# ctlab/metafast

Hardware: AMD Instinct MI355X
Metric: k-mers/s counted+graphed at k=31, 150 bp reads (higher is better)
Workload: dtype u64

## Files before the change

metafast_amd/csrc/mf_cc.hip:

```cpp
#include "mf_common.h"
#include "mf_nbr.h"
#include "mf_cc.h"
#include <algorithm>
#include <numeric>
#include <memory>

#define CC_NONE 0xFFFFFFFFu

__global__ void k_cc_adjacency(mf_index_view ix, const uint64_t *__restrict__ keys, uint64_t n,
                               int k, uint32_t *__restrict__ nbr) {
    uint64_t v = (uint64_t)blockIdx.x * blockDim.x + threadIdx.x;
    if (v >= n) return;
    const uint64_t kmask = (1ull << (2 * k)) - 1;
    const uint64_t x = keys[v];
    uint32_t out[8];
    uint32_t m_nf = 0, m_nl = 0;
    if (ix.skm_k) mf_skm_nbr_mins(x, k, &m_nf, &m_nl);
#pragma unroll
    for (uint32_t nuc = 0; nuc < 4; nuc++) {
        uint32_t idx, val;
        uint64_t y = ((x << 2) | nuc) & kmask;
        out[2 * nuc] = mf_index_find_ph(ix, mf_canon(y, k), ix.skm_k ? mf_skm_ph_right(y, k, m_nf) : 0u, &idx, &val) ? idx : CC_NONE;
        y = (x >> 2) | ((uint64_t)nuc << (2 * k - 2));
        out[2 * nuc + 1] = mf_index_find_ph(ix, mf_canon(y, k), ix.skm_k ? mf_skm_ph_left(y, k, m_nl) : 0u, &idx, &val) ? idx : CC_NONE;
    }
    uint4 *o = reinterpret_cast<uint4 *>(nbr + v * 8);
    o[0] = make_uint4(out[0], out[1], out[2], out[3]);
    o[1] = make_uint4(out[4], out[5], out[6], out[7]);
}

template <int MODE, int KT = 0>
__attribute__((amdgpu_waves_per_eu(KT ? 6 : 5, 8)))
__global__ __launch_bounds__(64 * NB_WAVES) void k_cc_adjacency_part(mf_index_view ix, const uint64_t *__restrict__ keys, const uint64_t *__restrict__ part_off,
                                                                   uint32_t np, int k_rt, uint32_t *__restrict__ nbr) {
    __shared__ nb_lds S;
    const int k = KT ? KT : k_rt;
    nb_for_each<MODE>(ix, keys, part_off, 0u, np, k, S, 0, 0u, [&](uint64_t v, uint64_t, const uint32_t (&idx)[8], uint32_t, uint32_t, bool have) {
        if (!have) return;
        uint4 *o = reinterpret_cast<uint4 *>(nbr + v * 8);
        o[0] = make_uint4(idx[0], idx[1], idx[2], idx[3]);
        o[1] = make_uint4(idx[4], idx[5], idx[6], idx[7]);
    });
}

__device__ __forceinline__ uint32_t cc_find(uint32_t *parent, uint32_t x) {
    for (;;) {
        uint32_t p = __hip_atomic_load(&parent[x], __ATOMIC_RELAXED, __HIP_MEMORY_SCOPE_AGENT);
        if (p == x) return x;
        uint32_t gp = __hip_atomic_load(&parent[p], __ATOMIC_RELAXED, __HIP_MEMORY_SCOPE_AGENT);
        if (gp != p) __hip_atomic_store(&parent[x], gp, __ATOMIC_RELAXED, __HIP_MEMORY_SCOPE_AGENT);
        x = gp;
    }
}
#define CC_TILE 1024
#define CC_LEDGE 2048
__global__ __launch_bounds__(256) void k_cc_hook_tile(const uint32_t *__restrict__ nbr, const uint8_t *__restrict__ alive, uint32_t *__restrict__ parent,
                                                      uint32_t *__restrict__ csize, unsigned long long *__restrict__ cweight, uint64_t n,
                                                      uint2 *__restrict__ edges, unsigned long long *__restrict__ ecount, uint64_t ecap) {
    __shared__ uint32_t lp[CC_TILE];
    __shared__ uint8_t la[CC_TILE];
    __shared__ uint2 le[CC_LEDGE];
    __shared__ uint32_t ln;
    __shared__ unsigned long long lbase;
    const uint64_t base = (uint64_t)blockIdx.x * CC_TILE;
    if (threadIdx.x == 0) ln = 0;
    for (uint32_t i = threadIdx.x; i < CC_TILE; i += blockDim.x) {
        lp[i] = i;
        const uint8_t al = base + i < n ? alive[base + i] : 0;
        la[i] = al;
        if (al) { csize[base + i] = 0; cweight[base + i] = 0; }
    }
    __syncthreads();
    auto find_l = [&](uint32_t x) -> uint32_t {
        for (;;) {
            const uint32_t p = *(volatile uint32_t *)&lp[x];
            if (p == x) return x;
            const uint32_t gp = *(volatile uint32_t *)&lp[p];
            if (gp != p) *(volatile uint32_t *)&lp[x] = gp;
            x = gp;
        }
    };
    for (uint32_t i = threadIdx.x; i < CC_TILE; i += blockDim.x) {
        if (!la[i]) continue;
        const uint64_t v = base + i;
        const uint4 *q = reinterpret_cast<const uint4 *>(nbr + v * 8);
        const uint4 a = q[0], b = q[1];
        const uint32_t nb[8] = {a.x, a.y, a.z, a.w, b.x, b.y, b.z, b.w};
#pragma unroll
        for (int j = 0; j < 8; j++) {
            const uint32_t u = nb[j];
            if (u == CC_NONE || u >= (uint32_t)v) continue;
            if (u < (uint32_t)base) {
                if (edges) { const uint32_t e = atomicAdd(&ln, 1u); if (e < (uint32_t)CC_LEDGE) le[e] = make_uint2((uint32_t)v, u); }
                continue;
// ... 797 lines not shown
        out[(size_t)i * n_samples + i] = 0.0;
        for (int j = i + 1; j < n_samples; j++) {
            double sumdiff = 0, sum = 0;
            const int64_t *a = vecs + (size_t)i * n_comp, *b = vecs + (size_t)j * n_comp;
            for (int p = 0; p < n_comp; p++) {
                double x = (double)a[p], y = (double)b[p];
                sumdiff += x > y ? x - y : y - x;
                sum += (x < 0 ? -x : x) + (y < 0 ? -y : y);
            }
            out[(size_t)i * n_samples + j] = out[(size_t)j * n_samples + i] = sumdiff / sum;
        }
    }
    return MF_OK;
}

struct dcc_query { uint64_t key; uint64_t src; };
struct dcc_kept_rec { uint32_t g, size; unsigned long long weight; };
#define DCC_NOKEY 0x7FFFFFFFFFFFFFFFull
struct mf_dcc {
    mf_ctx *ctx = nullptr; mf_table *t = nullptr; int k = 0, rank = 0, world = 1, lw = 0;
    uint32_t n = 0, n_total = 0; std::vector<uint32_t> base;
    mf_buf<uint32_t> nbr, parent, root, csize, groot;
    mf_buf<unsigned long long> cweight; mf_buf<uint8_t> alive;
    mf_buf<uint2> edges; mf_buf<unsigned long long> ecount; uint64_t ecap = 0;
    mf_buf<unsigned int> ctr;
    std::vector<uint64_t> qoff;
    mf_buf<unsigned long long> qcur;
    mf_buf<dcc_query> qflat; uint32_t nq = 0;
    mf_buf<uint32_t> xv, xu; mf_buf<uint8_t> xr, xalive; mf_buf<uint16_t> xval; uint64_t nx = 0;
    std::vector<uint64_t> xoff;
    mf_buf<uint32_t> pg, gsize; mf_buf<unsigned long long> gweight, gmin;
    mf_buf<uint64_t> mk; mf_buf<uint32_t> mg; uint64_t nm = 0;
    uint64_t nstat = 0, nkept_owned = 0; int level = 0;
    mf_buf<uint32_t> touched; mf_buf<uint2> hp; std::vector<uint64_t> xstart;
    mf_buf<dcc_kept_rec> keptbuf;
    mf_buf<uint64_t> gmk; mf_buf<uint2> gruns; uint64_t n_runs = 0;
    mf_buf<uint64_t> dseg; mf_buf<uint32_t> dbase;
};


static int dcc_log2(int w) { int l = 0; while ((1 << l) < w) l++; return l; }
#define DCC_SRC_MASK ((1ull << 56) - 1ull)
#define DCC_QCHUNK 512u
template <int MODE>
__global__ __launch_bounds__(64 * NB_WAVES) void k_dcc_adjacency_part(mf_index_view ix, const uint64_t *__restrict__ keys, const uint64_t *__restrict__ part_off,
                                                                    uint32_t p_lo, uint32_t p_hi, int k, int lw, uint32_t me, uint32_t *__restrict__ nbr,
                                                                    dcc_query *__restrict__ q, uint32_t qcap, unsigned int *__restrict__ qcount) {
    __shared__ nb_lds S;
    const uint64_t kmask = (1ull << (2 * k)) - 1;
    uint32_t qcur = 0, qend = 0;
    auto void_rest = [&]() {
        for (uint32_t i = qcur + mf_lane(); i < qend; i += 64) if (i < qcap) q[i].src = ~0ull;
    };
    nb_for_each<MODE>(ix, keys, part_off, p_lo, p_hi, k, S, lw, me, [&](uint64_t v, uint64_t x, const uint32_t (&idx)[8], uint32_t, uint32_t foreign, bool have) {
        if (have) {
            uint4 *o = reinterpret_cast<uint4 *>(nbr + v * 8);
            o[0] = make_uint4(idx[0], idx[1], idx[2], idx[3]);
            o[1] = make_uint4(idx[4], idx[5], idx[6], idx[7]);
        }
        const uint32_t cnt = have ? (uint32_t)__popc(foreign) : 0u;
        uint32_t tot;
        const uint32_t ex = mf_wave_excl_scan(cnt, &tot);
        if (!tot) return;
        if (qcur + tot > qend) {
            void_rest();
            uint32_t base = 0;
            const uint32_t ch = tot > DCC_QCHUNK ? tot : DCC_QCHUNK;
            if (mf_lane() == 0) base = atomicAdd(qcount, ch);
            qcur = (uint32_t)__builtin_amdgcn_readfirstlane((int)base);
            qend = qcur + ch;
        }
        uint32_t at = qcur + ex;
        qcur += tot;
        if (cnt) {
            uint32_t m_nf = 0, m_nl = 0;
            mf_skm_nbr_mins(x, k, &m_nf, &m_nl);
#pragma unroll
            for (uint32_t i = 0; i < 8; i++) {
                if (!((foreign >> i) & 1u)) continue;
                uint64_t y; uint32_t ph;
                const uint64_t c = nb_neighbour(x, k, kmask, i, m_nf, m_nl, &y, &ph);
                if (at < qcap) { q[at].key = c; q[at].src = (v * 8 + i) | ((uint64_t)(ph >> (32 - lw)) << 56); }
                at++;
            }
        }
    });
    void_rest();
}
template <bool FILL>
__global__ __launch_bounds__(256) void k_dcc_q_group(const dcc_query *__restrict__ q, uint32_t n, unsigned long long *__restrict__ cur, dcc_query *__restrict__ out) {
    __shared__ uint32_t cnt[64]; __shared__ unsigned long long base[64];
    if (threadIdx.x < 64) cnt[threadIdx.x] = 0;
    __syncthreads();
    const uint32_t per = 256 * 8, i0 = blockIdx.x * per;
    uint32_t o[8], pos[8];
#pragma unroll
    for (int j = 0; j < 8; j++) {
        const uint32_t i = i0 + (uint32_t)j * 256u + threadIdx.x;
        o[j] = 0xFFFFFFFFu;
        if (i < n) { o[j] = (uint32_t)(q[i].src >> 56); if (o[j] < 64u) pos[j] = atomicAdd(&cnt[o[j]], 1u); else o[j] = 0xFFFFFFFFu; }
    }
    __syncthreads();
    if (threadIdx.x < 64 && cnt[threadIdx.x]) base[threadIdx.x] = atomicAdd(&cur[threadIdx.x], (unsigned long long)cnt[threadIdx.x]);
    if (!FILL) return;
    __syncthreads();
#pragma unroll
    for (int j = 0; j < 8; j++) {
        const uint32_t i = i0 + (uint32_t)j * 256u + threadIdx.x;
        if (o[j] == 0xFFFFFFFFu) continue;
        dcc_query r = q[i];
        r.src &= DCC_SRC_MASK;
        out[base[o[j]] + pos[j]] = r;
    }
}
struct dcc_answer { uint64_t src; uint32_t lid; uint32_t val; };
__global__ void k_dcc_answer(mf_index_view ix, const dcc_query *__restrict__ q, uint64_t n, dcc_answer *__restrict__ a) {
    const uint64_t i = (uint64_t)blockIdx.x * blockDim.x + threadIdx.x;
    if (i >= n) return;
    uint32_t idx, val;
    const bool f = ix.slots && mf_index_find(ix, q[i].key, &idx, &val);
    a[i].src = q[i].src; a[i].lid = f ? idx : CC_NONE; a[i].val = f ? val : 0u;
}
__device__ __forceinline__ uint64_t dcc_reserve_by(unsigned long long *cur, uint32_t r, bool act, uint32_t *L) {
    unsigned long long *base = reinterpret_cast<unsigned long long *>(L + 64);
    __syncthreads();
    if (threadIdx.x < 64) L[threadIdx.x] = 0;
    __syncthreads();
    uint32_t pos = 0;
    if (act) pos = atomicAdd(&L[r], 1u);
    __syncthreads();
    if (threadIdx.x < 64 && L[threadIdx.x]) base[threadIdx.x] = atomicAdd(&cur[threadIdx.x], (unsigned long long)L[threadIdx.x]);
    __syncthreads();
    return act ? base[r] + pos : 0ull;
}
// ... 764 lines not shown
```

metafast_amd/csrc/mf_common.h:

```cpp
#pragma once
#include <hip/hip_runtime.h>
#include <stdint.h>
#include <stdarg.h>
#include <stdio.h>
#include <string.h>
#include <map>
#include <string>
#include <vector>
#include "../../include/metafast_hip.h"

int mf_set_error(const char *fmt, ...);

#define MF_HIP(call)                                                                              \
    do {                                                                                          \
        hipError_t e__ = (call);                                                                  \
        if (e__ != hipSuccess)                                                                    \
            return mf_set_error("%s failed: %s (%s:%d)", #call, hipGetErrorString(e__), __FILE__, \
                                __LINE__);                                                        \
    } while (0)
#define MF_TRY(call)                  \
    do {                              \
        int r__ = (call);             \
        if (r__ < 0) return r__;      \
    } while (0)
// ... 289 lines not shown
}

__device__ __forceinline__ uint32_t mf_block_excl_scan(uint32_t v, uint32_t *scratch, uint32_t *block_total) {
    uint32_t wtot;
    uint32_t ex = mf_wave_excl_scan(v, &wtot);
    int wave = threadIdx.x >> 6, nw = blockDim.x >> 6;
    __syncthreads();
    if (mf_lane() == 0) scratch[wave] = wtot;
    __syncthreads();
    if (threadIdx.x == 0) {
        uint32_t acc = 0;
        for (int i = 0; i < nw; i++) { uint32_t t = scratch[i]; scratch[i] = acc; acc += t; }
        scratch[16] = acc;
    }
    __syncthreads();
    uint32_t r = ex + scratch[wave];
    *block_total = scratch[16];
    return r;
}

__device__ __forceinline__ uint32_t mf_block_reserve(unsigned int *counter, uint32_t mine, uint32_t *scratch) {
    uint32_t tot;
    const uint32_t ex = mf_block_excl_scan(mine, scratch, &tot);
    if (threadIdx.x == 0) scratch[17] = tot ? atomicAdd(counter, tot) : 0u;
    __syncthreads();
    return scratch[17] + ex;
}

__host__ __device__ constexpr int mf_skm_m(int k) { return k <= 25 ? 13 : 15; }
#define MF_SKM_MIN_K 20
#define MF_SKM_BASES 50
__device__ __forceinline__ uint32_t mf_mmer_rc(uint32_t f, int M) {
    uint32_t r = __brev(~f);
    r = ((r & 0xAAAAAAAAu) >> 1) | ((r & 0x55555555u) << 1);
    return r >> (32 - 2 * M);
}
__host__ __device__ constexpr uint32_t mf_mmer_seed(int M) { return M == 13 ? 0x00B9107Fu : 0x051E6720u; }
__device__ __forceinline__ uint32_t mf_mmer_hash(uint32_t canon, int M) { return (canon ^ mf_mmer_seed(M)) * 0x9E3779B1u; }
__device__ __forceinline__ uint32_t mf_remix32(uint32_t h) { h ^= h >> 16; h *= 0x85EBCA6Bu; h ^= h >> 13; h *= 0xC2B2AE35u; return h ^ (h >> 16); }
__device__ __forceinline__ uint32_t mf_skm_ph(uint64_t key, int k) {
    const int M = mf_skm_m(k);
    const uint32_t mm = (1u << (2 * M)) - 1u;
    uint32_t f = (uint32_t)(key >> (2 * (k - M))) & mm, r = mf_mmer_rc(f, M);
    uint32_t best = mf_mmer_hash(f < r ? f : r, M);
    for (int j = k - M - 1; j >= 0; j--) {
        const uint32_t b = (uint32_t)(key >> (2 * j)) & 3u;
        f = ((f << 2) | b) & mm;
        r = (r >> 2) | ((3u - b) << (2 * M - 2));
        const uint32_t h = mf_mmer_hash(f < r ? f : r, M);
        best = h < best ? h : best;
    }
    return mf_remix32(best);
}
__device__ __forceinline__ void mf_skm_nbr_mins(uint64_t x, int k, uint32_t *no_first, uint32_t *no_last, uint32_t *own = nullptr) {
    const int M = mf_skm_m(k);
    const uint32_t mm = (1u << (2 * M)) - 1u;
    uint32_t f = (uint32_t)(x >> (2 * (k - M))) & mm, r = mf_mmer_rc(f, M);
    uint32_t h = mf_mmer_hash(f < r ? f : r, M);
    uint32_t a = 0xFFFFFFFFu, b = h;
    for (int j = k - M - 1; j >= 0; j--) {
        const uint32_t c = (uint32_t)(x >> (2 * j)) & 3u;
        f = ((f << 2) | c) & mm;
        r = (r >> 2) | ((3u - c) << (2 * M - 2));
        h = mf_mmer_hash(f < r ? f : r, M);
        a = h < a ? h : a;
        if (j > 0) b = h < b ? h : b;
    }
    *no_first = a; *no_last = b;
    if (own) *own = h < b ? h : b;
}
__device__ __forceinline__ uint32_t mf_skm_mn_right(uint64_t y, int k, uint32_t no_first_of_x) {
    const int M = mf_skm_m(k);
    const uint32_t f = (uint32_t)y & ((1u << (2 * M)) - 1u), r = mf_mmer_rc(f, M);
    const uint32_t h = mf_mmer_hash(f < r ? f : r, M);
    return h < no_first_of_x ? h : no_first_of_x;
}
__device__ __forceinline__ uint32_t mf_skm_mn_left(uint64_t y, int k, uint32_t no_last_of_x) {
    const int M = mf_skm_m(k);
    const uint32_t f = (uint32_t)(y >> (2 * (k - M))) & ((1u << (2 * M)) - 1u), r = mf_mmer_rc(f, M);
    const uint32_t h = mf_mmer_hash(f < r ? f : r, M);
    return h < no_last_of_x ? h : no_last_of_x;
}
__device__ __forceinline__ uint32_t mf_skm_ph_right(uint64_t y, int k, uint32_t no_first_of_x) { return mf_remix32(mf_skm_mn_right(y, k, no_first_of_x)); }
__device__ __forceinline__ uint32_t mf_skm_ph_left(uint64_t y, int k, uint32_t no_last_of_x) { return mf_remix32(mf_skm_mn_left(y, k, no_last_of_x)); }
struct mf_slot { uint64_t key; uint32_t idx; uint32_t val; };
int mf_sort_pairs(mf_ctx *ctx, const uint64_t *d_keys_in, const uint16_t *d_vals_in, uint64_t n, int key_bits, uint64_t *d_keys_out,
                  uint16_t *d_vals_out);
int mf_sort_u32_pairs(mf_ctx *ctx, const uint32_t *d_keys_in, const uint32_t *d_vals_in, uint64_t n, int bits, uint32_t *d_keys_out,
                      uint32_t *d_vals_out);
int mf_sort_u32_u64(mf_ctx *ctx, const uint32_t *d_keys_in, const uint64_t *d_vals_in, uint64_t n, int bits, uint32_t *d_keys_out,
                    uint64_t *d_vals_out);
int mf_sort_u64_u32(mf_ctx *ctx, const uint64_t *d_keys_in, const uint32_t *d_vals_in, uint64_t n, int bits, uint64_t *d_keys_out, uint32_t *d_vals_out);
int mf_sort_u64_u64(mf_ctx *ctx, const uint64_t *d_keys_in, const uint64_t *d_vals_in, uint64_t n, int bits, uint64_t *d_keys_out, uint64_t *d_vals_out);
int mf_sort_u64_u64_pingpong(mf_ctx *ctx, uint64_t *k0, uint64_t *v0, uint64_t n, int first_bit, int bits, uint64_t *k1, uint64_t *v1, int *in_second);
int mf_sort_u64_u64_range(mf_ctx *ctx, const uint64_t *d_keys_in, const uint64_t *d_vals_in, uint64_t n, int first_bit, int bits, uint64_t *d_keys_out, uint64_t *d_vals_out);
int mf_select_by(mf_ctx *ctx, const uint64_t *keys, const uint16_t *sel, const uint16_t *vals, uint64_t n, int thr, mf_buf<uint64_t> &ok,
                 mf_buf<uint16_t> &oc, uint64_t *n_out);
int mf_sum_counts(mf_ctx *ctx, const uint16_t *d_counts, uint64_t n, uint64_t *total);
int mf_table_load_kmers_sum(mf_ctx *ctx, const char *const *files, int nfiles, int freq_threshold, int k, mf_table **out, uint64_t *freq_sum);
int mf_sort_kmers_by_comp(mf_ctx *ctx, const uint32_t *d_comp, const uint64_t *d_kmers, uint64_t n, int key_bits, uint32_t n_comps,
                          uint64_t *d_out);
__host__ __device__ __forceinline__ uint64_t mf_interior(uint64_t x, uint64_t rcx, int k) {
    const uint64_t WM = (1ull << (2 * k - 4)) - 1ull;
    const uint64_t w = (x >> 2) & WM, rw = (rcx >> 2) & WM;
    return w < rw ? w : rw;
}
__host__ __device__ __forceinline__ uint64_t mf_cidx_hkey(uint64_t key, uint32_t skm_k) {
    return skm_k >= 3u ? mf_interior(key, mf_revcomp(key, (int)skm_k), (int)skm_k) : key;
}
__device__ __forceinline__ bool mf_index_find_ph(const mf_index_view &ix, uint64_t key, uint32_t ph, uint32_t *idx, uint32_t *val) {
    if (ix.compact) {
        const uint64_t h = mf_phash(mf_cidx_hkey(key, ix.skm_k));
        const uint64_t part = ix.skm_k ? (uint64_t)(ph >> (32 - ix.part_bits)) : (h >> (64 - ix.part_bits));
        const ulonglong2 d = *reinterpret_cast<const ulonglong2 *>(&ix.dir[2 * part]);
        const uint32_t *__restrict__ reg = reinterpret_cast<const uint32_t *>(ix.slots) + (d.x >> 6);
        const uint32_t rmask = (1u << (uint32_t)(d.x & 63ull)) - 1u, hs = mf_pslot(h), tag = hs >> MF_CIDX_REL_BITS;
        uint32_t s = hs & rmask;
        for (;;) {
            const uint32_t v = reg[s];
            if (v == MF_CIDX_EMPTY) return false;
            if ((v >> MF_CIDX_REL_BITS) == tag) {
                const uint64_t i = d.y + (uint64_t)(v & ((1u << MF_CIDX_REL_BITS) - 1u));
// ... 169 lines not shown
```

metafast_amd/csrc/mf_nbr.h:

```cpp
#pragma once
#include "mf_common.h"
#ifdef __HIPCC__
#define NB_SLOTS 1024
#define NB_CAP 352
#define NB_WAVES 4
#define NB_NONE 0xFFFFFFFFu

#define NB_RQ 64
struct nb_lds {
    uint64_t key[NB_WAVES][NB_CAP];
    uint64_t rq_pa[NB_WAVES][NB_RQ], rq_pb[NB_WAVES][NB_RQ];
    uint32_t rq_mn[NB_WAVES][NB_RQ], rq_meta[NB_WAVES][NB_RQ];
    uint32_t slot[NB_WAVES][NB_SLOTS / 2];
};

__device__ __forceinline__ uint64_t nb_neighbour(uint64_t x, uint64_t rcx, int k, uint64_t kmask, uint32_t i, uint32_t m_nf, uint32_t m_nl, uint64_t *oriented, uint32_t *ph) {
    const uint32_t nuc = i >> 1;
    uint64_t y, r;
    if (i & 1u) { y = (x >> 2) | ((uint64_t)nuc << (2 * k - 2)); r = ((rcx << 2) | (uint64_t)(3u - nuc)) & kmask; *ph = mf_skm_ph_left(y, k, m_nl); }
    else { y = ((x << 2) | nuc) & kmask; r = (rcx >> 2) | ((uint64_t)(3u - nuc) << (2 * k - 2)); *ph = mf_skm_ph_right(y, k, m_nf); }
    *oriented = y;
    return y < r ? y : r;
}
__device__ __forceinline__ uint64_t nb_neighbour(uint64_t x, int k, uint64_t kmask, uint32_t i, uint32_t m_nf, uint32_t m_nl, uint64_t *oriented, uint32_t *ph) {
    return nb_neighbour(x, mf_revcomp(x, k), k, kmask, i, m_nf, m_nl, oriented, ph);
}
#define NB_BIGCAP (NB_CAP * NB_WAVES)
__device__ __forceinline__ uint32_t nb_hash(uint64_t key) { return ((uint32_t)key ^ (uint32_t)(key >> 29)) * 0x9E3779B1u; }
__device__ __forceinline__ uint64_t nb_interior(uint64_t x, uint64_t rcx, int k) {
    const uint64_t WM = (1ull << (2 * k - 4)) - 1ull;
    const uint64_t w = (x >> 2) & WM, rw = (rcx >> 2) & WM;
    return w < rw ? w : rw;
}
template <int MODE, typename F>
__device__ __forceinline__ void nb_for_each(const mf_index_view &ix, const uint64_t *__restrict__ keys, const uint64_t *__restrict__ part_off,
                                            uint32_t p_lo, uint32_t np, int k, nb_lds &S, int lw, uint32_t me, F &&emit) {
    constexpr bool BIG = MODE == 2;
    constexpr uint32_t SLOTS = BIG ? (uint32_t)(NB_SLOTS * NB_WAVES) : (uint32_t)NB_SLOTS;
    constexpr int HSHIFT = BIG ? 20 : 22;
    constexpr int POSBITS = BIG ? 11 : 9;
    constexpr uint32_t POSMASK = (1u << POSBITS) - 1u;
    constexpr int TSHIFT = HSHIFT - (16 - POSBITS);
    constexpr uint32_t TAGMASK = (1u << (16 - POSBITS)) - 1u;
    const uint32_t wave = threadIdx.x >> 6, lane = threadIdx.x & 63u;
    const uint32_t first = BIG ? blockIdx.x : blockIdx.x * NB_WAVES + wave, stride = BIG ? gridDim.x : gridDim.x * NB_WAVES;
    const uint64_t kmask = (1ull << (2 * k)) - 1;
    uint64_t *hk = BIG ? &S.key[0][0] : S.key[wave]; uint32_t *hw = BIG ? &S.slot[0][0] : S.slot[wave];
    const uint16_t *hs = reinterpret_cast<const uint16_t *>(hw);
    uint64_t *qa = S.rq_pa[wave], *qb = S.rq_pb[wave]; uint32_t *qm = S.rq_mn[wave], *qt = S.rq_meta[wave];
    const uint32_t tl = BIG ? threadIdx.x : lane, tn = BIG ? (uint32_t)(64 * NB_WAVES) : 64u;
    auto wave_sync = [&]() { __builtin_amdgcn_fence(__ATOMIC_RELEASE, "wavefront"); __builtin_amdgcn_wave_barrier(); __builtin_amdgcn_fence(__ATOMIC_ACQUIRE, "wavefront"); };
    auto team_sync = [&]() { if (BIG) __syncthreads(); else wave_sync(); };
    for (uint32_t p = p_lo + first; p < np; p += stride) {
        const uint64_t lo = part_off[p], hi = part_off[p + 1];
        const uint32_t n = (uint32_t)(hi - lo);
        if (n == 0) continue;
        const bool mid = n > (uint32_t)NB_CAP && n <= (uint32_t)NB_BIGCAP;
        if (MODE == 1 && mid) continue;
        if (MODE == 2 && !mid) continue;
        const bool local = BIG || n <= (uint32_t)NB_CAP;
        if (local) {
            for (uint32_t s = tl; s < SLOTS / 2; s += tn) hw[s] = 0xFFFFFFFFu;
            team_sync();
            for (uint32_t j = tl; j < n; j += tn) {
                const uint64_t x = keys[lo + j];
                hk[j] = x;
                const uint32_t h = nb_hash(nb_interior(x, mf_revcomp(x, k), k));
                const uint32_t ent = (((h >> TSHIFT) & TAGMASK) << POSBITS) | j;
                uint32_t s = h >> HSHIFT;
                for (;;) {
                    uint32_t *w = &hw[s >> 1];
                    const uint32_t sh = (s & 1u) * 16u;
                    const uint32_t old = __atomic_load_n(w, __ATOMIC_RELAXED);
                    if (((old >> sh) & 0xFFFFu) != 0xFFFFu) { s = (s + 1u) & (SLOTS - 1u); continue; }
                    if (atomicCAS(w, old, (old & ~(0xFFFFu << sh)) | (ent << sh)) == old) break;
                }
            }
            team_sync();
        }
        constexpr uint32_t JSTEP = BIG ? (uint32_t)(64 * NB_WAVES) : 64u;
        for (uint32_t j0 = BIG ? wave * 64u : 0u; j0 < n; j0 += JSTEP) {
            const uint32_t j = j0 + lane;
            const bool have = j < n;
            const uint64_t x = have ? (local ? hk[j] : keys[lo + j]) : 0ull;
            uint32_t m_nf = 0, m_nl = 0, m_own = 0;
            mf_skm_nbr_mins(x, k, &m_nf, &m_nl, &m_own);
            uint32_t remote = 0, foreign = 0, flip = 0;
            uint32_t phs[8];
            const uint64_t rcx = mf_revcomp(x, k);
            const int M = mf_skm_m(k);
            const uint32_t MM = (1u << (2 * M)) - 1u;
#pragma unroll
            for (uint32_t i = 0; i < 8; i++) {
                const uint32_t nuc = i >> 1;
                const uint32_t f = (i & 1u) ? (((uint32_t)(x >> (2 * (k - M) + 2)) & (MM >> 2)) | (nuc << (2 * M - 2))) : ((((uint32_t)x << 2) | nuc) & MM);
                const uint32_t r = mf_mmer_rc(f, M), h = mf_mmer_hash(f < r ? f : r, M), mo = (i & 1u) ? m_nl : m_nf;
                phs[i] = h < mo ? h : mo;
                if (have && lw && (mf_remix32(phs[i]) >> (32 - lw)) != me) foreign |= 1u << i;
                else if (have && !(local && phs[i] == m_own)) remote |= 1u << i;
            }
            uint32_t lead[2], grouped = 0, nreq = 0;
#pragma unroll
            for (uint32_t side = 0; side < 2; side++) {
                const uint32_t rem = (remote >> side) & 0x55u;
                lead[side] = 0;
                bool same = true;
#pragma unroll
                for (int c = 3; c >= 0; c--) if ((rem >> (2 * c)) & 1u) lead[side] = phs[2 * c + side];
#pragma unroll
                for (uint32_t c = 0; c < 4; c++) if (((rem >> (2 * c)) & 1u) && phs[2 * c + side] != lead[side]) same = false;
                if (same) grouped |= 1u << side;
                nreq += rem ? (same ? 1u : (uint32_t)__popc(rem)) : 0u;
            }
            uint32_t R;
            const uint32_t rbase = mf_wave_excl_scan(nreq, &R);
            uint32_t idx[8];
#pragma unroll
            for (uint32_t i = 0; i < 8; i++) idx[i] = NB_NONE;
            {
                const uint64_t LM = kmask >> 2;
                uint32_t at = rbase;
#pragma unroll
                for (uint32_t side = 0; side < 2; side++) {
                    const uint32_t rem = (remote >> side) & 0x55u;
                    if (!rem) continue;
                    const uint64_t pa = side ? (rcx & LM) : (x & LM), pb = side ? (x >> 2) : (rcx >> 2);
                    uint32_t want4 = 0;
#pragma unroll
                    for (uint32_t c = 0; c < 4; c++) want4 |= ((rem >> (2 * c)) & 1u) << c;
                    if ((grouped >> side) & 1u) {
                        if (at < (uint32_t)NB_RQ) { qa[at] = pa; qb[at] = pb; qm[at] = lead[side]; qt[at] = side | (want4 << 1); }
                        else {
                            uint32_t o4[4], rv;
                            mf_index_walk_side(ix, mf_remix32(lead[side]), pa, pb, side, want4, k, o4, &rv);
#pragma unroll
                            for (uint32_t c = 0; c < 4; c++) if ((want4 >> c) & 1u) { idx[2 * c + side] = o4[c]; flip |= ((rv >> c) & 1u) << (2 * c + side); }
                        }
                        at++;
                    } else {
#pragma unroll
                        for (uint32_t c = 0; c < 4; c++) {
                            if (!((want4 >> c) & 1u)) continue;
                            if (at < (uint32_t)NB_RQ) { qa[at] = pa; qb[at] = pb; qm[at] = phs[2 * c + side]; qt[at] = side | (1u << (c + 1)); }
                            else { uint32_t o4[4], rv; mf_index_walk_side(ix, mf_remix32(phs[2 * c + side]), pa, pb, side, 1u << c, k, o4, &rv); idx[2 * c + side] = o4[c]; flip |= ((rv >> c) & 1u) << (2 * c + side); }
                            at++;
                        }
                    }
                }
            }
            static_assert(NB_RQ <= 64, "one request per lane");
            const uint32_t Rl = R < (uint32_t)NB_RQ ? R : (uint32_t)NB_RQ;
            ulonglong2 dent = make_ulonglong2(0ull, 0ull);
            if (R) {
                wave_sync();
                if (lane < Rl && ix.compact) dent = mf_index_side_dir(ix, mf_remix32(qm[lane]));
            }
            if (local) {
                const uint64_t LM = kmask >> 2, WM = kmask >> 4;
                const uint32_t nloc = ~(remote | foreign);
#pragma unroll
                for (uint32_t side = 0; side < 2; side++) {
                    if (have && (nloc & (0x55u << side))) {
                        const uint64_t w = side ? (x >> 4) : (x & WM), rw = side ? (rcx & WM) : (rcx >> 4);
                        const uint64_t pa = side ? (rcx & LM) : (x & LM);
                        const uint64_t pb = side ? (x >> 2) : (rcx >> 2);
                        const uint32_t h = nb_hash(w < rw ? w : rw), tag = (h >> TSHIFT) & TAGMASK;
                        uint32_t s = h >> HSHIFT;
                        for (;;) {
                            const uint32_t v = hs[s];
                            if (v == 0xFFFFu) break;
                            if ((v >> POSBITS) == tag) {
                                const uint64_t K = hk[v & POSMASK];
                                const bool ma = (K >> 2) == pa, mb = (K & LM) == pb, fwd = side ? mb : ma;
                                const uint32_t ca = ((uint32_t)K & 3u) ^ (side ? 3u : 0u), cb = (uint32_t)(K >> (2 * k - 2)) ^ (side ? 0u : 3u);
                                const uint32_t c = (ma || mb) ? (fwd ? (side ? cb : ca) : (side ? ca : cb)) : 4u;
                                const uint32_t at = (uint32_t)lo + (v & POSMASK);
#pragma unroll
                                for (uint32_t q = 0; q < 4; q++)
                                    if (c == q && ((nloc >> (2 * q + side)) & 1u)) { idx[2 * q + side] = at; flip = (flip & ~(1u << (2 * q + side))) | ((fwd ? 0u : 1u) << (2 * q + side)); }
                            }
                            s = (s + 1u) & (SLOTS - 1u);
                        }
                    }
                }
            }
            if (R) {
                if (lane < Rl) {
                    uint32_t o4[4], rv = 0;
                    const uint32_t meta = qt[lane];
                    if (ix.compact) mf_index_walk_side_d(ix, dent, qa[lane], qb[lane], meta & 1u, meta >> 1, k, o4, &rv);
                    else mf_index_walk_side(ix, mf_remix32(qm[lane]), qa[lane], qb[lane], meta & 1u, meta >> 1, k, o4, &rv);
                    uint32_t *ans = reinterpret_cast<uint32_t *>(&qa[lane]), *ans2 = reinterpret_cast<uint32_t *>(&qb[lane]);
                    ans[0] = o4[0]; ans[1] = o4[1]; ans2[0] = o4[2]; ans2[1] = o4[3]; qt[lane] = rv;
                }
                wave_sync();
                uint32_t at = rbase;
#pragma unroll
                for (uint32_t side = 0; side < 2; side++) {
                    const uint32_t rem = (remote >> side) & 0x55u;
                    if (!rem) continue;
#pragma unroll
                    for (uint32_t c = 0; c < 4; c++) {
                        if (!((rem >> (2 * c)) & 1u)) continue;
                        if (at < (uint32_t)NB_RQ) {
                            idx[2 * c + side] = c < 2 ? reinterpret_cast<const uint32_t *>(&qa[at])[c] : reinterpret_cast<const uint32_t *>(&qb[at])[c - 2];
                            flip |= ((qt[at] >> c) & 1u) << (2 * c + side);
                        }
                        if (!((grouped >> side) & 1u)) at++;
                    }
                    if ((grouped >> side) & 1u) at++;
                }
                wave_sync();
            }
            emit(lo + j, x, idx, flip, foreign, have);
        }
        team_sync();
    }
}
#endif
```

metafast_amd/csrc/mf_unitig.hip:

```cpp
#include "mf_common.h"
#include "mf_nbr.h"
#include "mf_unitig.h"
#include "mf_wide.h"
#include <algorithm>
#include <numeric>

#define UT_NONE 0xFFFFFFFFu
#define UT_CODE_NONE 4u
#define UT_CODE_MANY 5u
#define UT_WALK_CHUNK 4096

__global__ void k_ut_flags(mf_index_view ix, ut_arrays A) {
    uint64_t i = (uint64_t)blockIdx.x * blockDim.x + threadIdx.x;
    if (i >= A.n) return;
    const int k = A.k;
    const uint64_t kmask = (k == 32) ? ~0ull : ((1ull << (2 * k)) - 1);
    const uint64_t x = A.gk[i];
    uint32_t rcode = UT_CODE_NONE, lcode = UT_CODE_NONE, ridx = UT_NONE, lidx = UT_NONE, ror = 0, lor = 0;
    uint32_t m_nf = 0, m_nl = 0;
    if (ix.skm_k) mf_skm_nbr_mins(x, k, &m_nf, &m_nl);
#pragma unroll
    for (uint32_t nuc = 0; nuc < 4; nuc++) {
        uint64_t y = ((x << 2) | nuc) & kmask;
        uint64_t ry = mf_revcomp(y, k);
        uint64_t c = y < ry ? y : ry;
        uint32_t idx, val;
        if (mf_index_find_ph(ix, c, ix.skm_k ? mf_skm_ph_right(y, k, m_nf) : 0u, &idx, &val)) {
            if (rcode == UT_CODE_NONE) { rcode = nuc; ridx = idx; ror = (c != y); }
            else rcode = UT_CODE_MANY;
        }
    }
#pragma unroll
    for (uint32_t nuc = 0; nuc < 4; nuc++) {
        uint64_t y = (x >> 2) | ((uint64_t)nuc << (2 * k - 2));
        uint64_t ry = mf_revcomp(y, k);
        uint64_t c = y < ry ? y : ry;
        uint32_t idx, val;
        if (mf_index_find_ph(ix, c, ix.skm_k ? mf_skm_ph_left(y, k, m_nl) : 0u, &idx, &val)) {
            if (lcode == UT_CODE_NONE) { lcode = nuc; lidx = idx; lor = (c != y); }
            else lcode = UT_CODE_MANY;
        }
    }
    A.info[i] = (uint8_t)(rcode | (lcode << 3) | (ror << 6) | (lor << 7));
    if (A.pal) A.pal[i] = (uint8_t)(mf_revcomp(x, k) == x);
    A.ridx[i] = ridx;
    A.lidx[i] = lidx;
}

template <int MODE, int KT = 0>
#ifndef NB_NOFORCE
__attribute__((amdgpu_waves_per_eu((KT == 0 || KT == 25 || KT == 29) ? 5 : 6, 8)))
#endif
__global__ __launch_bounds__(64 * NB_WAVES) void k_ut_flags_part(mf_index_view ix, ut_arrays A, const uint64_t *__restrict__ part_off, uint32_t np) {
    __shared__ nb_lds S;
    const int k = KT ? KT : A.k;
    nb_for_each<MODE>(ix, A.gk, part_off, 0u, np, k, S, 0, 0u, [&](uint64_t i, uint64_t x, const uint32_t (&idx)[8], uint32_t flip, uint32_t, bool have) {
        if (!have) return;
        uint32_t rcode = UT_CODE_NONE, lcode = UT_CODE_NONE, ridx = UT_NONE, lidx = UT_NONE, ror = 0, lor = 0;
#pragma unroll
        for (uint32_t nuc = 0; nuc < 4; nuc++) {
            if (idx[2 * nuc] != NB_NONE) {
                if (rcode == UT_CODE_NONE) { rcode = nuc; ridx = idx[2 * nuc]; ror = (flip >> (2 * nuc)) & 1u; }
                else rcode = UT_CODE_MANY;
            }
            if (idx[2 * nuc + 1] != NB_NONE) {
                if (lcode == UT_CODE_NONE) { lcode = nuc; lidx = idx[2 * nuc + 1]; lor = (flip >> (2 * nuc + 1)) & 1u; }
                else lcode = UT_CODE_MANY;
            }
        }
        A.info[i] = (uint8_t)(rcode | (lcode << 3) | (ror << 6) | (lor << 7));
        if (A.pal) A.pal[i] = (uint8_t)(mf_revcomp(x, k) == x);
        A.ridx[i] = ridx;
        A.lidx[i] = lidx;
    });
}

__device__ __forceinline__ bool ut_r_unique(uint8_t info, uint32_t o) { return ((o ? (info >> 3) : info) & 7u) < 4u; }
__device__ __forceinline__ bool ut_l_unique(uint8_t info, uint32_t o) { return ((o ? info : (info >> 3)) & 7u) < 4u; }
__device__ __forceinline__ uint32_t ut_node(const ut_arrays &A, uint32_t idx, uint32_t strand) {
    if (A.pal && A.pal[idx]) strand = 0;
    return idx * 2u + strand;
}
__device__ __forceinline__ uint32_t ut_right_node(const ut_arrays &A, uint32_t i, uint32_t o, uint8_t info) {
    return o ? ut_node(A, A.lidx[i], ((info >> 7) & 1u) ^ 1u) : ut_node(A, A.ridx[i], (info >> 6) & 1u);
}
__device__ __forceinline__ uint32_t ut_left_node(const ut_arrays &A, uint32_t i, uint32_t o, uint8_t info) {
    return o ? ut_node(A, A.ridx[i], ((info >> 6) & 1u) ^ 1u) : ut_node(A, A.lidx[i], (info >> 7) & 1u);
}

template <bool W>
__global__ __launch_bounds__(1024) void k_ut_links(ut_arrays A) {
    const uint64_t i = (uint64_t)blockIdx.x * blockDim.x + threadIdx.x;
    bool st0 = false, st1 = false;
    if (i < A.n) {
        const uint8_t info = A.info[i];
        const bool pal_i = A.pal && A.pal[i];
        const bool ru = ut_r_unique(info, 0), lu = ut_l_unique(info, 0);
        uint32_t ri = 0, li = 0;
        uint8_t iR = 0, iL = 0;
        bool palR = false, palL = false;
        if (ru) { ri = A.ridx[i]; iR = A.info[ri]; palR = A.pal && A.pal[ri]; }
        if (lu) { li = A.lidx[i]; iL = A.info[li]; palL = A.pal && A.pal[li]; }
        const uint32_t ror = (info >> 6) & 1u, lor = (info >> 7) & 1u;
        uint32_t succ0 = UT_NONE, succ1 = UT_NONE;
        if (ru) { const uint32_t sd = palR ? 0u : ror; if (ut_l_unique(iR, sd)) succ0 = ri * 2u + sd; }
        { bool has_in = false; if (lu) has_in = ut_r_unique(iL, palL ? 0u : lor); st0 = !has_in; }
        if (!pal_i) {
            if (lu) { const uint32_t sd = palL ? 0u : (lor ^ 1u); if (ut_l_unique(iL, sd)) succ1 = li * 2u + sd; }
            bool has_in = false;
            if (ru) has_in = ut_r_unique(iR, palR ? 0u : (ror ^ 1u));
            st1 = !has_in;
        }
        const uint64_t x = A.gk[i];
        const uint64_t cnt = (uint64_t)A.gv[i] << 32;
        const uint64_t w0 = (uint64_t)succ0 | cnt | ((x & 3ull) << 48);
        const int fsh = 2 * A.k - 2;
        const uint32_t first = W ? (uint32_t)((fsh >= 64 ? A.ghi[i] >> (fsh - 64) : x >> fsh) & 3ull) : (uint32_t)((x >> fsh) & 3ull);
        const uint64_t w1 = (uint64_t)succ1 | cnt | ((uint64_t)(3u - first) << 48);
        *reinterpret_cast<ulonglong2 *>(&A.node[2 * i]) = make_ulonglong2(w0, w1);
    }
    __shared__ uint32_t wave_base[16];
    __shared__ uint32_t block_base;
    const unsigned long long b0 = __ballot(st0), b1 = __ballot(st1);
    const int wave = threadIdx.x >> 6;
    if (mf_lane() == 0) wave_base[wave] = (uint32_t)(__popcll(b0) + __popcll(b1));
    __syncthreads();
// ... 879 lines not shown
```

Before: 92.62 billion.

## Template neighbour walk on a result sink and reuse reverse complement for minimizers

The neighbour-enumeration loop now takes a sink type, so the unitig flags kernel keeps only per-side counts and the first hit instead of an 8-entry index array plus flip mask. This cuts register pressure, and the unitig kernel's waves-per-EU hint is raised to 6 for all k. Minimizer computation now pulls m-mers directly from x and its precomputed reverse complement, and neighbour m-mer hashes are built from per-side base templates rather than recomputing mf_mmer_rc. The forced occupancy risks spills for some k values, and the minimizer rewrite changes the arithmetic pattern.

After: 92.90 billion, median of 3. No clear change (+0.3%).

```diff
diff --git a/metafast_amd/csrc/mf_cc.hip b/metafast_amd/csrc/mf_cc.hip
--- a/metafast_amd/csrc/mf_cc.hip
+++ b/metafast_amd/csrc/mf_cc.hip
@@ -35,11 +35,11 @@
                                                                    uint32_t np, int k_rt, uint32_t *__restrict__ nbr) {
     __shared__ nb_lds S;
     const int k = KT ? KT : k_rt;
-    nb_for_each<MODE>(ix, keys, part_off, 0u, np, k, S, 0, 0u, [&](uint64_t v, uint64_t, const uint32_t (&idx)[8], uint32_t, uint32_t, bool have) {
+    nb_for_each<MODE, nb_sink_all>(ix, keys, part_off, 0u, np, k, S, 0, 0u, [&](uint64_t v, uint64_t, uint64_t, const nb_sink_all &N, uint32_t, bool have) {
         if (!have) return;
         uint4 *o = reinterpret_cast<uint4 *>(nbr + v * 8);
-        o[0] = make_uint4(idx[0], idx[1], idx[2], idx[3]);
-        o[1] = make_uint4(idx[4], idx[5], idx[6], idx[7]);
+        o[0] = make_uint4(N.idx[0], N.idx[1], N.idx[2], N.idx[3]);
+        o[1] = make_uint4(N.idx[4], N.idx[5], N.idx[6], N.idx[7]);
     });
 }
 
@@ -943,11 +943,11 @@
     auto void_rest = [&]() {
         for (uint32_t i = qcur + mf_lane(); i < qend; i += 64) if (i < qcap) q[i].src = ~0ull;
     };
-    nb_for_each<MODE>(ix, keys, part_off, p_lo, p_hi, k, S, lw, me, [&](uint64_t v, uint64_t x, const uint32_t (&idx)[8], uint32_t, uint32_t foreign, bool have) {
+    nb_for_each<MODE, nb_sink_all>(ix, keys, part_off, p_lo, p_hi, k, S, lw, me, [&](uint64_t v, uint64_t x, uint64_t rcx, const nb_sink_all &N, uint32_t foreign, bool have) {
         if (have) {
             uint4 *o = reinterpret_cast<uint4 *>(nbr + v * 8);
-            o[0] = make_uint4(idx[0], idx[1], idx[2], idx[3]);
-            o[1] = make_uint4(idx[4], idx[5], idx[6], idx[7]);
+            o[0] = make_uint4(N.idx[0], N.idx[1], N.idx[2], N.idx[3]);
+            o[1] = make_uint4(N.idx[4], N.idx[5], N.idx[6], N.idx[7]);
         }
         const uint32_t cnt = have ? (uint32_t)__popc(foreign) : 0u;
         uint32_t tot;
@@ -965,12 +965,12 @@
         qcur += tot;
         if (cnt) {
             uint32_t m_nf = 0, m_nl = 0;
-            mf_skm_nbr_mins(x, k, &m_nf, &m_nl);
+            mf_skm_nbr_mins(x, rcx, k, &m_nf, &m_nl);
 #pragma unroll
             for (uint32_t i = 0; i < 8; i++) {
                 if (!((foreign >> i) & 1u)) continue;
                 uint64_t y; uint32_t ph;
-                const uint64_t c = nb_neighbour(x, k, kmask, i, m_nf, m_nl, &y, &ph);
+                const uint64_t c = nb_neighbour(x, rcx, k, kmask, i, m_nf, m_nl, &y, &ph);
                 if (at < qcap) { q[at].key = c; q[at].src = (v * 8 + i) | ((uint64_t)(ph >> (32 - lw)) << 56); }
                 at++;
             }
diff --git a/metafast_amd/csrc/mf_common.h b/metafast_amd/csrc/mf_common.h
--- a/metafast_amd/csrc/mf_common.h
+++ b/metafast_amd/csrc/mf_common.h
@@ -365,22 +365,37 @@
     }
     return mf_remix32(best);
 }
+__device__ __forceinline__ uint32_t mf_mmer_at(uint64_t x, int j, int M) { return (uint32_t)(x >> (2 * j)) & ((1u << (2 * M)) - 1u); }
+__device__ __forceinline__ uint32_t mf_mmer_rc_at(uint64_t rcx, int j, int k, int M) { return mf_mmer_at(rcx, k - M - j, M); }
+__device__ __forceinline__ uint32_t mf_mmer_hash_at(uint64_t x, uint64_t rcx, int j, int k, int M) {
+    const uint32_t f = mf_mmer_at(x, j, M), r = mf_mmer_rc_at(rcx, j, k, M);
+    return mf_mmer_hash(f < r ? f : r, M);
+}
+struct mf_nbr_mmers { uint32_t f, r; };
+__device__ __forceinline__ mf_nbr_mmers mf_nbr_mmers_right(uint64_t x, uint64_t rcx, int k, int M) {
+    return {((uint32_t)x << 2) & ((1u << (2 * M)) - 1u), (uint32_t)(rcx >> (2 * (k - M + 1)))};
+}
+__device__ __forceinline__ mf_nbr_mmers mf_nbr_mmers_left(uint64_t x, uint64_t rcx, int k, int M) {
+    return {(uint32_t)(x >> (2 * (k - M + 1))), ((uint32_t)rcx << 2) & ((1u << (2 * M)) - 1u)};
+}
+__device__ __forceinline__ uint32_t mf_nbr_mmer_hash(const mf_nbr_mmers &B, uint32_t side, uint32_t c, int M) {
+    const uint32_t f = B.f | (c << (side ? 2 * M - 2 : 0)), r = B.r | ((3u - c) << (side ? 0 : 2 * M - 2));
+    return mf_mmer_hash(f < r ? f : r, M);
+}
+__device__ __forceinline__ void mf_skm_nbr_mins(uint64_t x, uint64_t rcx, int k, uint32_t *no_first, uint32_t *no_last, uint32_t *own = nullptr) {
+    const int M = mf_skm_m(k);
+    const uint32_t first = mf_mmer_hash_at(x, rcx, k - M, k, M), last = mf_mmer_hash_at(x, rcx, 0, k, M);
+    uint32_t mid = 0xFFFFFFFFu;
+    for (int j = k - M - 1; j > 0; j--) {
+        const uint32_t h = mf_mmer_hash_at(x, rcx, j, k, M);
+        mid = h < mid ? h : mid;
+    }
+    const uint32_t b = first < mid ? first : mid;
+    *no_first = last < mid ? last : mid; *no_last = b;
+    if (own) *own = last < b ? last : b;
+}
 __device__ __forceinline__ void mf_skm_nbr_mins(uint64_t x, int k, uint32_t *no_first, uint32_t *no_last, uint32_t *own = nullptr) {
-    const int M = mf_skm_m(k);
-    const uint32_t mm = (1u << (2 * M)) - 1u;
-    uint32_t f = (uint32_t)(x >> (2 * (k - M))) & mm, r = mf_mmer_rc(f, M);
-    uint32_t h = mf_mmer_hash(f < r ? f : r, M);
-    uint32_t a = 0xFFFFFFFFu, b = h;
-    for (int j = k - M - 1; j >= 0; j--) {
-        const uint32_t c = (uint32_t)(x >> (2 * j)) & 3u;
-        f = ((f << 2) | c) & mm;
-        r = (r >> 2) | ((3u - c) << (2 * M - 2));
-        h = mf_mmer_hash(f < r ? f : r, M);
-        a = h < a ? h : a;
-        if (j > 0) b = h < b ? h : b;
-    }
-    *no_first = a; *no_last = b;
-    if (own) *own = h < b ? h : b;
+    mf_skm_nbr_mins(x, mf_revcomp(x, k), k, no_first, no_last, own);
 }
 __device__ __forceinline__ uint32_t mf_skm_mn_right(uint64_t y, int k, uint32_t no_first_of_x) {
     const int M = mf_skm_m(k);
diff --git a/metafast_amd/csrc/mf_nbr.h b/metafast_amd/csrc/mf_nbr.h
--- a/metafast_amd/csrc/mf_nbr.h
+++ b/metafast_amd/csrc/mf_nbr.h
@@ -25,6 +25,27 @@
 __device__ __forceinline__ uint64_t nb_neighbour(uint64_t x, int k, uint64_t kmask, uint32_t i, uint32_t m_nf, uint32_t m_nl, uint64_t *oriented, uint32_t *ph) {
     return nb_neighbour(x, mf_revcomp(x, k), k, kmask, i, m_nf, m_nl, oriented, ph);
 }
+struct nb_sink_all {
+    uint32_t idx[8];
+    __device__ __forceinline__ void clear() {
+#pragma unroll
+        for (uint32_t i = 0; i < 8; i++) idx[i] = NB_NONE;
+    }
+    __device__ __forceinline__ void put(uint32_t side, uint32_t c, uint32_t at, uint32_t) {
+#pragma unroll
+        for (uint32_t q = 0; q < 4; q++) if (c == q) idx[2 * q + side] = at;
+    }
+};
+struct nb_sink_sides {
+    uint32_t cnt[2], cr[2], at[2];
+    __device__ __forceinline__ void clear() { cnt[0] = cnt[1] = 0u; cr[0] = cr[1] = 8u; at[0] = at[1] = NB_NONE; }
+    __device__ __forceinline__ void put(uint32_t side, uint32_t c, uint32_t where, uint32_t rev) {
+        const uint32_t v = (c << 1) | rev;
+        at[side] = v < cr[side] ? where : at[side];
+        cr[side] = v < cr[side] ? v : cr[side];
+        cnt[side]++;
+    }
+};
 #define NB_BIGCAP (NB_CAP * NB_WAVES)
 __device__ __forceinline__ uint32_t nb_hash(uint64_t key) { return ((uint32_t)key ^ (uint32_t)(key >> 29)) * 0x9E3779B1u; }
 __device__ __forceinline__ uint64_t nb_interior(uint64_t x, uint64_t rcx, int k) {
@@ -32,7 +53,7 @@
     const uint64_t w = (x >> 2) & WM, rw = (rcx >> 2) & WM;
     return w < rw ? w : rw;
 }
-template <int MODE, typename F>
+template <int MODE, typename SINK, typename F>
 __device__ __forceinline__ void nb_for_each(const mf_index_view &ix, const uint64_t *__restrict__ keys, const uint64_t *__restrict__ part_off,
                                             uint32_t p_lo, uint32_t np, int k, nb_lds &S, int lw, uint32_t me, F &&emit) {
     constexpr bool BIG = MODE == 2;
@@ -83,18 +104,16 @@
             const uint32_t j = j0 + lane;
             const bool have = j < n;
             const uint64_t x = have ? (local ? hk[j] : keys[lo + j]) : 0ull;
+            const uint64_t rcx = mf_revcomp(x, k);
             uint32_t m_nf = 0, m_nl = 0, m_own = 0;
-            mf_skm_nbr_mins(x, k, &m_nf, &m_nl, &m_own);
-            uint32_t remote = 0, foreign = 0, flip = 0;
+            mf_skm_nbr_mins(x, rcx, k, &m_nf, &m_nl, &m_own);
+            uint32_t remote = 0, foreign = 0;
             uint32_t phs[8];
-            const uint64_t rcx = mf_revcomp(x, k);
             const int M = mf_skm_m(k);
-            const uint32_t MM = (1u << (2 * M)) - 1u;
+            const mf_nbr_mmers nbm[2] = {mf_nbr_mmers_right(x, rcx, k, M), mf_nbr_mmers_left(x, rcx, k, M)};
 #pragma unroll
             for (uint32_t i = 0; i < 8; i++) {
-                const uint32_t nuc = i >> 1;
-                const uint32_t f = (i & 1u) ? (((uint32_t)(x >> (2 * (k - M) + 2)) & (MM >> 2)) | (nuc << (2 * M - 2))) : ((((uint32_t)x << 2) | nuc) & MM);
-                const uint32_t r = mf_mmer_rc(f, M), h = mf_mmer_hash(f < r ? f : r, M), mo = (i & 1u) ? m_nl : m_nf;
+                const uint32_t h = mf_nbr_mmer_hash(nbm[i & 1u], i & 1u, i >> 1, M), mo = (i & 1u) ? m_nl : m_nf;
                 phs[i] = h < mo ? h : mo;
                 if (have && lw && (mf_remix32(phs[i]) >> (32 - lw)) != me) foreign |= 1u << i;
                 else if (have && !(local && phs[i] == m_own)) remote |= 1u << i;
@@ -114,9 +133,8 @@
             }
             uint32_t R;
             const uint32_t rbase = mf_wave_excl_scan(nreq, &R);
-            uint32_t idx[8];
-#pragma unroll
-            for (uint32_t i = 0; i < 8; i++) idx[i] = NB_NONE;
+            SINK sink;
+            sink.clear();
             {
                 const uint64_t LM = kmask >> 2;
                 uint32_t at = rbase;
@@ -134,7 +152,7 @@
                             uint32_t o4[4], rv;
                             mf_index_walk_side(ix, mf_remix32(lead[side]), pa, pb, side, want4, k, o4, &rv);
 #pragma unroll
-                            for (uint32_t c = 0; c < 4; c++) if ((want4 >> c) & 1u) { idx[2 * c + side] = o4[c]; flip |= ((rv >> c) & 1u) << (2 * c + side); }
+                            for (uint32_t c = 0; c < 4; c++) if (o4[c] != NB_NONE) sink.put(side, c, o4[c], (rv >> c) & 1u);
                         }
                         at++;
                     } else {
@@ -142,7 +160,7 @@
                         for (uint32_t c = 0; c < 4; c++) {
                             if (!((want4 >> c) & 1u)) continue;
                             if (at < (uint32_t)NB_RQ) { qa[at] = pa; qb[at] = pb; qm[at] = phs[2 * c + side]; qt[at] = side | (1u << (c + 1)); }
-                            else { uint32_t o4[4], rv; mf_index_walk_side(ix, mf_remix32(phs[2 * c + side]), pa, pb, side, 1u << c, k, o4, &rv); idx[2 * c + side] = o4[c]; flip |= ((rv >> c) & 1u) << (2 * c + side); }
+                            else { uint32_t o4[4], rv; mf_index_walk_side(ix, mf_remix32(phs[2 * c + side]), pa, pb, side, 1u << c, k, o4, &rv); if (o4[c] != NB_NONE) sink.put(side, c, o4[c], (rv >> c) & 1u); }
                             at++;
                         }
                     }
@@ -157,7 +175,7 @@
             }
             if (local) {
                 const uint64_t LM = kmask >> 2, WM = kmask >> 4;
-                const uint32_t nloc = ~(remote | foreign);
+                const uint32_t nloc = ~(remote | foreign), nloc_w = nloc & 0xFFu;
 #pragma unroll
                 for (uint32_t side = 0; side < 2; side++) {
                     if (have && (nloc & (0x55u << side))) {
@@ -174,10 +192,7 @@
                                 const bool ma = (K >> 2) == pa, mb = (K & LM) == pb, fwd = side ? mb : ma;
                                 const uint32_t ca = ((uint32_t)K & 3u) ^ (side ? 3u : 0u), cb = (uint32_t)(K >> (2 * k - 2)) ^ (side ? 0u : 3u);
                                 const uint32_t c = (ma || mb) ? (fwd ? (side ? cb : ca) : (side ? ca : cb)) : 4u;
-                                const uint32_t at = (uint32_t)lo + (v & POSMASK);
-#pragma unroll
-                                for (uint32_t q = 0; q < 4; q++)
-                                    if (c == q && ((nloc >> (2 * q + side)) & 1u)) { idx[2 * q + side] = at; flip = (flip & ~(1u << (2 * q + side))) | ((fwd ? 0u : 1u) << (2 * q + side)); }
+                                if ((nloc_w >> (2 * c + side)) & 1u) sink.put(side, c, (uint32_t)lo + (v & POSMASK), fwd ? 0u : 1u);
                             }
                             s = (s + 1u) & (SLOTS - 1u);
                         }
@@ -199,20 +214,29 @@
                 for (uint32_t side = 0; side < 2; side++) {
                     const uint32_t rem = (remote >> side) & 0x55u;
                     if (!rem) continue;
-#pragma unroll
-                    for (uint32_t c = 0; c < 4; c++) {
-                        if (!((rem >> (2 * c)) & 1u)) continue;
+                    if ((grouped >> side) & 1u) {
                         if (at < (uint32_t)NB_RQ) {
-                            idx[2 * c + side] = c < 2 ? reinterpret_cast<const uint32_t *>(&qa[at])[c] : reinterpret_cast<const uint32_t *>(&qb[at])[c - 2];
-                            flip |= ((qt[at] >> c) & 1u) << (2 * c + side);
-                        }
-                        if (!((grouped >> side) & 1u)) at++;
+                            const uint2 a01 = *reinterpret_cast<const uint2 *>(&qa[at]), a23 = *reinterpret_cast<const uint2 *>(&qb[at]);
+                            const uint32_t a4[4] = {a01.x, a01.y, a23.x, a23.y}, rv = qt[at];
+#pragma unroll
+                            for (uint32_t c = 0; c < 4; c++) if (a4[c] != NB_NONE) sink.put(side, c, a4[c], (rv >> c) & 1u);
+                        }
+                        at++;
+                    } else {
+#pragma unroll
+                        for (uint32_t c = 0; c < 4; c++) {
+                            if (!((rem >> (2 * c)) & 1u)) continue;
+                            if (at < (uint32_t)NB_RQ) {
+                                const uint32_t a = c < 2 ? reinterpret_cast<const uint32_t *>(&qa[at])[c] : reinterpret_cast<const uint32_t *>(&qb[at])[c - 2];
+                                if (a != NB_NONE) sink.put(side, c, a, (qt[at] >> c) & 1u);
+                            }
+                            at++;
+                        }
                     }
-                    if ((grouped >> side) & 1u) at++;
                 }
                 wave_sync();
             }
-            emit(lo + j, x, idx, flip, foreign, have);
+            emit(lo + j, x, rcx, sink, foreign, have);
         }
         team_sync();
     }
diff --git a/metafast_amd/csrc/mf_unitig.hip b/metafast_amd/csrc/mf_unitig.hip
--- a/metafast_amd/csrc/mf_unitig.hip
+++ b/metafast_amd/csrc/mf_unitig.hip
@@ -49,29 +49,19 @@
 
 template <int MODE, int KT = 0>
 #ifndef NB_NOFORCE
-__attribute__((amdgpu_waves_per_eu((KT == 0 || KT == 25 || KT == 29) ? 5 : 6, 8)))
+__attribute__((amdgpu_waves_per_eu(6, 8)))
 #endif
 __global__ __launch_bounds__(64 * NB_WAVES) void k_ut_flags_part(mf_index_view ix, ut_arrays A, const uint64_t *__restrict__ part_off, uint32_t np) {
     __shared__ nb_lds S;
     const int k = KT ? KT : A.k;
-    nb_for_each<MODE>(ix, A.gk, part_off, 0u, np, k, S, 0, 0u, [&](uint64_t i, uint64_t x, const uint32_t (&idx)[8], uint32_t flip, uint32_t, bool have) {
+    static_assert(UT_CODE_NONE == 4u && UT_NONE == NB_NONE, "nb_sink_sides' empty record is the flags' 'none'");
+    nb_for_each<MODE, nb_sink_sides>(ix, A.gk, part_off, 0u, np, k, S, 0, 0u, [&](uint64_t i, uint64_t x, uint64_t rcx, const nb_sink_sides &N, uint32_t, bool have) {
         if (!have) return;
-        uint32_t rcode = UT_CODE_NONE, lcode = UT_CODE_NONE, ridx = UT_NONE, lidx = UT_NONE, ror = 0, lor = 0;
-#pragma unroll
-        for (uint32_t nuc = 0; nuc < 4; nuc++) {
-            if (idx[2 * nuc] != NB_NONE) {
-                if (rcode == UT_CODE_NONE) { rcode = nuc; ridx = idx[2 * nuc]; ror = (flip >> (2 * nuc)) & 1u; }
-                else rcode = UT_CODE_MANY;
-            }
-            if (idx[2 * nuc + 1] != NB_NONE) {
-                if (lcode == UT_CODE_NONE) { lcode = nuc; lidx = idx[2 * nuc + 1]; lor = (flip >> (2 * nuc + 1)) & 1u; }
-                else lcode = UT_CODE_MANY;
-            }
-        }
-        A.info[i] = (uint8_t)(rcode | (lcode << 3) | (ror << 6) | (lor << 7));
-        if (A.pal) A.pal[i] = (uint8_t)(mf_revcomp(x, k) == x);
-        A.ridx[i] = ridx;
-        A.lidx[i] = lidx;
+        const uint32_t rcode = N.cnt[0] > 1u ? UT_CODE_MANY : N.cr[0] >> 1, lcode = N.cnt[1] > 1u ? UT_CODE_MANY : N.cr[1] >> 1;
+        A.info[i] = (uint8_t)(rcode | (lcode << 3) | ((N.cr[0] & 1u) << 6) | ((N.cr[1] & 1u) << 7));
+        if (A.pal) A.pal[i] = (uint8_t)(rcx == x);
+        A.ridx[i] = N.at[0];
+        A.lidx[i] = N.at[1];
     });
 }
 
```
